# tmtlakmal/acme

Hardware: NVIDIA B200
Metric: learner_updates_per_sec_dqn_atari_b256 (higher is better)
Workload: dtype bf16 tensor-core operands (activations, weight shadows, back-propagated gradients), f32 accumulate, f32 master weights, weight gradients and optimizer

## Files before the change

acme_b200/_capi.py:

```python

from __future__ import annotations

import ctypes as C
import os

_LIB_PATH = os.path.join(os.path.dirname(os.path.abspath(__file__)), 'lib', 'libb200rl.so')

c_i32, c_i64, c_u64, c_f32, c_f64, c_vp, c_int = (C.c_int32, C.c_int64, C.c_uint64, C.c_float,
                                                  C.c_double, C.c_void_p, C.c_int)


class ReplayCfg(C.Structure):
  _fields_ = [('max_items', c_i64), ('slot_capacity', c_i64), ('obs_bytes', c_i32),
              ('act_bytes', c_i32), ('max_window', c_i32), ('shard_count', c_i32),
              ('shard_rank', c_i32), ('device', c_i32), ('stage_slots', c_i32),
              ('frame_stack', c_i32), ('gamma', c_f32), ('reserved_f', c_f32), ('alpha', c_f64)]


class DpCfg(C.Structure):
  _fields_ = [('world', c_i32), ('rank', c_i32), ('device', c_i32), ('reserved', c_i32), ('n_params', c_i64)]


class ConvGeom(C.Structure):
  _fields_ = [(n, c_i32) for n in ('B', 'H', 'W', 'C', 'kh', 'kw', 'stride', 'pad_top',
# ... 65 lines not shown
                                  c_int, c_vp, c_i64, c_vp]),
    'b200rl_linear_dgrad': (c_int, [c_i32, c_i32, c_i32, c_vp, c_i32, c_vp, c_vp, c_i32, c_vp, c_int,
                                    c_int, c_vp, c_i64, c_vp]),
    'b200rl_linear_wgrad': (c_int, [c_i32, c_i32, c_i32, c_vp, c_i32, c_vp, c_i32, c_vp, c_vp, c_int,
                                    c_vp, c_i64, c_vp]),
    'b200rl_act_bwd': (c_int, [c_i64, c_vp, c_vp, c_int, c_vp]),
    'b200rl_duelling_fwd': (c_int, [c_i32, c_i32, c_vp, c_vp, c_vp, c_vp]),
    'b200rl_duelling_bwd': (c_int, [c_i32, c_i32, c_vp, c_vp, c_vp, c_vp]),
    'b200rl_duelling_head_fwd': (c_int, [c_i32, c_i32, c_i32, c_vp, c_i32, c_vp, c_vp, c_vp, c_vp, c_vp, c_vp, c_vp, c_vp]),
    'b200rl_duelling_head_bwd': (c_int, [c_i32, c_i32, c_i32, c_vp, c_vp, c_i32, c_vp, c_vp, c_vp, c_vp, c_vp, c_i32, c_vp, c_vp,
                                          c_vp, c_vp, c_vp, c_i64, c_vp]),
    'b200rl_dqn_head_td': (c_int, [c_i32, c_i32, c_i32, c_vp, c_vp, c_vp, c_i32, c_vp, c_vp, c_vp, c_vp, c_vp, c_vp, c_vp, c_vp,
                                   c_vp, c_vp, c_vp, c_vp, c_f32, c_f32, c_f64, c_f32, c_vp, c_f32, c_i32, c_vp, c_vp, c_vp, c_vp,
                                   c_vp, c_vp, c_vp, c_vp, c_vp, c_vp, c_vp, c_i32, c_i32, c_vp]),
    'b200rl_mean': (c_int, [c_i32, c_vp, c_vp, c_vp]),
    'b200rl_duelling_head_wgrad': (c_int, [c_i32, c_i32, c_i32, c_vp, c_vp, c_vp, c_i32, c_vp, c_vp, c_vp, c_vp, c_vp, c_i64, c_vp]),
    'b200rl_bf16_from_f32': (c_int, [c_i64, c_vp, c_vp, c_vp]),
    'b200rl_conv2d_rows_bf16_bytes': (c_i64, [C.POINTER(ConvGeom)]),
    'b200rl_conv2d_rows_bf16_from_u8': (c_int, [c_vp, C.POINTER(ConvGeom), c_vp, c_i64, c_vp]),
    'b200rl_conv2d_fwd_bf16': (c_int, [c_vp, c_int, c_vp, c_vp, c_vp, c_int, C.POINTER(ConvGeom), c_int, c_vp, c_i64, c_vp]),
    'b200rl_conv2d_wgrad_bf16': (c_int, [c_vp, c_int, c_vp, c_vp, c_vp, C.POINTER(ConvGeom), c_vp, c_i64, c_vp]),
    'b200rl_conv2d_dgrad_bf16': (c_int, [c_vp, c_vp, c_vp, c_int, C.POINTER(ConvGeom), c_vp, c_int, c_int, c_vp]),
    'b200rl_linear_fwd_bf16': (c_int, [c_i32, c_i32, c_i32, c_vp, c_i32, c_vp, c_vp, c_vp, c_i32, c_int, c_int, c_vp, c_i64, c_vp]),
    'b200rl_linear_dgrad_bf16': (c_int, [c_i32, c_i32, c_i32, c_vp, c_i32, c_vp, c_vp, c_i32, c_int, c_vp, c_int, c_int, c_vp,
                                         c_i64, c_vp]),
    'b200rl_colsum_bf16': (c_int, [c_i32, c_i32, c_vp, c_i32, c_vp, c_vp, c_i64, c_vp]),
    'b200rl_linear_wgrad_bf16': (c_int, [c_i32, c_i32, c_i32, c_vp, c_i32, c_vp, c_i32, c_vp, c_vp, c_vp, c_i64, c_vp]),
    'b200rl_layernorm_tanh_fwd': (c_int, [c_i32, c_i32, c_vp, c_vp, c_vp, c_f32, c_vp, c_vp, c_vp, c_vp]),
    'b200rl_layernorm_tanh_bwd': (c_int, [c_i32, c_i32, c_vp, c_vp, c_vp, c_vp, c_vp, c_vp, c_vp, c_vp, c_vp]),
    'b200rl_tanh_to_spec_fwd': (c_int, [c_i32, c_i32, c_vp, c_vp, c_vp, c_vp, c_vp]),
    'b200rl_tanh_to_spec_bwd': (c_int, [c_i32, c_i32, c_vp, c_vp, c_vp, c_vp, c_vp]),
    'b200rl_concat2': (c_int, [c_i32, c_i32, c_i32, c_vp, c_vp, c_vp, c_vp]),
    'b200rl_split_second': (c_int, [c_i32, c_i32, c_i32, c_vp, c_vp, c_vp]),
    'b200rl_workspace_bytes': (c_i64, [c_i64]),
    'b200rl_conv2d_rows_bytes': (c_i64, [C.POINTER(ConvGeom)]),
    'b200rl_conv2d_rows_from_u8': (c_int, [c_vp, C.POINTER(ConvGeom), c_vp, c_i64, c_vp]),
    'b200rl_dp_create': (c_int, [C.POINTER(c_vp), C.POINTER(DpCfg)]),
    'b200rl_dp_destroy': (c_int, [c_vp]),
    'b200rl_dp_buffers': (c_int, [c_vp, C.POINTER(c_vp), C.POINTER(c_vp)]),
    'b200rl_dp_export': (c_int, [c_vp, c_vp]),
    'b200rl_dp_import': (c_int, [c_vp, c_i32, c_vp]),
    'b200rl_dp_max_f64': (c_int, [c_vp, c_vp, c_vp, c_vp]),
    'b200rl_dp_adam': (c_int, [c_vp, c_i64, c_i64, c_vp, c_vp, c_vp, C.c_float, C.c_double, C.c_double, C.c_float, c_int,
                               c_i32, c_i32, c_vp]),
    'b200rl_dp_reduce_adam_ce': (c_int, [c_vp, c_i64, c_i64, c_vp, c_vp, c_vp, C.c_float, C.c_double, C.c_double, C.c_float, c_int,
                                 c_i32, c_vp, c_i32, c_vp]),
    'b200rl_dp_region_bytes': (c_i64, [c_i64]),
    'b200rl_dp_create_external': (c_int, [C.POINTER(c_vp), C.POINTER(DpCfg), C.POINTER(c_vp), c_vp]),
# ... 71 lines not shown
```

acme_b200/csrc/gemm_bf16.cu:

```cuda
#include <algorithm>
#include <cstdlib>

#include <cuda.h>
#include <cuda_bf16.h>

#include "common.cuh"
#include "gemm_common.cuh"
#include "tc_common.cuh"
#include "tma_common.cuh"

namespace b200rl {

typedef __nv_bfloat16 bf16;
constexpr int HBM_ROWS = 128, H_THREADS = 192;

__device__ unsigned long long* g_h_timeline = nullptr;
__device__ __forceinline__ void h_mark(int slot, int cta) {
  if (g_h_timeline && (int)(blockIdx.x + blockIdx.y * gridDim.x) == cta && blockIdx.z == 0) {
    unsigned long long t;
    asm volatile("mov.u64 %0, %%globaltimer;" : "=l"(t));
    g_h_timeline[slot] = t;
  }
}

// ... 415 lines not shown
      rc = launch_h_pers<KE, BM, BN, true>(ma, mb, epi, M, N, K, kps, splits, res_b, stream, conv);
    else
      rc = launch_h_pers<KE, BM, BN, false>(ma, mb, epi, M, N, K, kps, splits, 0, stream, conv);
    if (rc) return rc;
    if (splits > 1) return launch_splitk_finish(epi, M, N, splits, stream);
    return B200RL_OK;
  }
  dim3 grid(ceil_div(N, BN), ceil_div(M, HBM_ROWS), splits);
  constexpr int smem = STAGES * STAGE + 1024;
  static bool attr = false;
  if (!attr) {
    B200RL_CUDA_OK(cudaFuncSetAttribute(hgemm_kernel<KE, AM, BM, BN, STAGES>, cudaFuncAttributeMaxDynamicSharedMemorySize, smem));
    attr = true;
  }
  epi.pdl_late = pdl_late_mode();
  B200RL_CUDA_OK(launch_pdl(hgemm_kernel<KE, AM, BM, BN, STAGES>, grid, dim3(H_THREADS), smem, stream, ma, mb, epi, M, N, K, kps, conv));
  B200RL_LAUNCH_OK();
  if (splits > 1) return launch_splitk_finish(epi, M, N, splits, stream);
  return B200RL_OK;
}
static const ConvA kNoConv{0, 0, 0, 0, 0, 0, 0, 0, 0, 0};
static int bn_for(int N) { return N <= 32 ? 32 : (N <= 64 ? 64 : 128); }

static Epilogue make_epi(void* out, int ldo, const float* bias, int act, const void* mask, int ldmask, int mask_act,
                         int transpose, int out_bf16, int mask_bf16, float scale) {
  Epilogue e{(float*)out, ldo, bias, act, (const float*)mask, ldmask, mask_act, nullptr, transpose, out_bf16, mask_bf16, scale};
  return e;
}

int h_linear_fwd(int M, int N, int K, const bf16* x, int ldx, const bf16* w, const float* bias, void* y, int ldy, int act,
                 int out_bf16, void* ws, int64_t wsb, cudaStream_t s) {
  if (!ok16(x, ldx) || !ok16(w, K) || K < 64) return 1;
  const int BN = bn_for(N);
  CUtensorMap ma, mb;
  if (!make_map_h(&ma, x, M, K, ldx, 64, HBM_ROWS) || !make_map_h(&mb, w, N, K, K, 64, BN)) return 1;
  Epilogue e = make_epi(y, ldy, bias, act, nullptr, 0, 0, 0, out_bf16, 0, 0.f);
  if (BN == 32) return launch_h<64, 0, 0, 32>(ma, mb, e, M, N, K, ws, wsb, s, kNoConv);
  if (BN == 64) return launch_h<64, 0, 0, 64>(ma, mb, e, M, N, K, ws, wsb, s, kNoConv);
  return launch_h<64, 0, 0, 128>(ma, mb, e, M, N, K, ws, wsb, s, kNoConv);
}
int h_linear_dgrad(int M, int N, int K, const bf16* dy, int lddy, const bf16* w, void* dx, int lddx, const void* mask,
                   int ldmask, int mask_act, int out_bf16, int mask_bf16, void* ws, int64_t wsb, cudaStream_t s) {
  if (!ok16(dy, lddy) || !ok16(w, K) || N < 64 || K % 64 != 0) return 1;
  int BN = K >= 128 ? 128 : 64;
  if (BN == 128 && ceil_div(M, HBM_ROWS) * ceil_div(K, 128) < kNumSMs) BN = 64;
  CUtensorMap ma, mb;
  if (!make_map_h(&ma, dy, M, N, lddy, 64, HBM_ROWS) || !make_map_h(&mb, w, N, K, K, 64, 64)) return 1;
  Epilogue e = make_epi(dx, lddx, nullptr, 0, mask, ldmask, mask_act, 0, out_bf16, mask_bf16, 0.f);
  return BN == 64 ? launch_h<64, 0, 1, 64>(ma, mb, e, M, K, N, ws, wsb, s, kNoConv, false)
                  : launch_h<64, 0, 1, 128>(ma, mb, e, M, K, N, ws, wsb, s, kNoConv, false);
}
int launch_colsum_bf16(int M, int N, const bf16* x, int ld, float* out, void* ws, int64_t ws_bytes, cudaStream_t stream);

int h_linear_wgrad(int M, int N, int K, const bf16* dy, int lddy, const bf16* x, int ldx, float* dw, float* db, void* ws,
                   int64_t wsb, cudaStream_t s) {
  if (!ok16(dy, lddy) || !ok16(x, ldx) || N % 64 != 0 || K % 64 != 0) return 1;
  const int BN = K >= 128 ? 128 : 64;
  CUtensorMap ma, mb;
  if (!make_map_h(&ma, dy, M, N, lddy, 64, 64) || !make_map_h(&mb, x, M, K, ldx, 64, 64)) return 1;
  Epilogue e = make_epi(dw, K, nullptr, 0, nullptr, 0, 0, 0, 0, 0, 0.f);
  int rc = BN == 64 ? launch_h<64, 1, 1, 64>(ma, mb, e, N, K, M, ws, wsb, s, kNoConv)
                    : launch_h<64, 1, 1, 128>(ma, mb, e, N, K, M, ws, wsb, s, kNoConv);
  if (rc) return rc;
  if (db) return launch_colsum_bf16(M, N, dy, lddy, db, ws, wsb, s);
  return B200RL_OK;
}

int h_conv_fwd(const bf16* x, const bf16* w, const float* bias, void* y, const b200rl_conv_geom& g, int act, int out_bf16,
               void* ws, int64_t wsb, cudaStream_t s) {
  const int M = g.B * g.OH * g.OW, K = g.kh * g.kw * g.C;
  if ((g.C != 32 && g.C % 64 != 0) || !ok16(x, g.C) || !ok16(w, K) || (g.Cout != 32 && g.Cout != 64 && g.Cout != 128)) return 1;
  const int KE = g.C == 32 ? 32 : 64;
  CUtensorMap ma, mb;
// ... 490 lines not shown
```

acme_b200/csrc/layers_api.cu:

```cuda
#include <cuda_bf16.h>

#include "common.cuh"

namespace b200rl {
int simt_linear_fwd(int M, int N, int K, const float* x, int ldx, const float* w, const float* bias, float* y,
                    int ldy, int act, void* ws, int64_t wsb, cudaStream_t s);
int simt_linear_dgrad(int M, int N, int K, const float* dy, int lddy, const float* w, float* dx, int lddx,
                      const float* mask, int ldmask, int mask_act, void* ws, int64_t wsb, cudaStream_t s);
int simt_linear_wgrad(int M, int N, int K, const float* dy, int lddy, const float* x, int ldx, float* dw, float* db,
                      void* ws, int64_t wsb, cudaStream_t s);
int simt_conv_fwd(const void* x, int x_u8, const float* w, const float* bias, float* y, const b200rl_conv_geom& g,
                  int act, void* ws, int64_t wsb, cudaStream_t s);
int simt_conv_wgrad(const void* x, int x_u8, const float* dy, float* dw, float* db, const b200rl_conv_geom& g,
                    void* ws, int64_t wsb, cudaStream_t s);
int simt_conv_dgrad(const float* dy, const float* w, float* dx, const b200rl_conv_geom& g, const float* mask,
                    int mask_act, void* ws, int64_t wsb, cudaStream_t s);
int tc_linear_fwd(int M, int N, int K, const float* x, int ldx, const float* w, const float* bias, float* y,
                  int ldy, int act, void* ws, int64_t wsb, cudaStream_t s);
int tc_linear_dgrad(int M, int N, int K, const float* dy, int lddy, const float* w, float* dx, int lddx,
                    const float* mask, int ldmask, int mask_act, void* ws, int64_t wsb, cudaStream_t s);
int tc_linear_wgrad(int M, int N, int K, const float* dy, int lddy, const float* x, int ldx, float* dw, float* db,
                    void* ws, int64_t wsb, cudaStream_t s);
int tc_conv_fwd(const void* x, int x_u8, const float* w, const float* bias, float* y, const b200rl_conv_geom& g,
                int act, void* ws, int64_t wsb, cudaStream_t s);
// ... 5 lines not shown
                   int ldy, int act, void* ws, int64_t wsb, cudaStream_t s);
int tma_linear_dgrad(int M, int N, int K, const float* dy, int lddy, const float* w, float* dx, int lddx,
                     const float* mask, int ldmask, int mask_act, void* ws, int64_t wsb, cudaStream_t s);
int tma_linear_wgrad(int M, int N, int K, const float* dy, int lddy, const float* x, int ldx, float* dw, float* db,
                     void* ws, int64_t wsb, cudaStream_t s);
int tma_conv_fwd(const float* x, const float* w, const float* bias, float* y, const b200rl_conv_geom& g, int act,
                 void* ws, int64_t wsb, cudaStream_t s);
int tma_conv_wgrad(const float* x, const float* dy, float* dw, float* db, const b200rl_conv_geom& g, void* ws, int64_t wsb,
                   cudaStream_t s);
int tma_conv_dgrad(const float* dy, const float* w, float* dx, const b200rl_conv_geom& g, const float* mask, int mask_act,
                   void* ws, int64_t wsb, cudaStream_t s);
int tma_conv_fwd_u8(const uint8_t* x, const float* w, const float* bias, float* y, const b200rl_conv_geom& g, int act,
                    void* ws, int64_t wsb, cudaStream_t s);
int tma_conv_wgrad_u8(const uint8_t* x, const float* dy, float* dw, float* db, const b200rl_conv_geom& g, void* ws, int64_t wsb,
                      cudaStream_t s);
int64_t tma_rows_bytes(const b200rl_conv_geom& g);
int tma_rows_from_u8(const uint8_t* x, const b200rl_conv_geom& g, float* rows, int64_t bytes, cudaStream_t s);
int tma_conv_fwd_rows(const float* rows, const float* w, const float* bias, float* y, const b200rl_conv_geom& g, int act,
                      void* ws, int64_t wsb, cudaStream_t s);
int tma_conv_wgrad_rows(const float* rows, const float* dy, float* dw, float* db, const b200rl_conv_geom& g, void* ws,
                        int64_t wsb, cudaStream_t s);
int h_linear_fwd(int M, int N, int K, const __nv_bfloat16* x, int ldx, const __nv_bfloat16* w, const float* bias, void* y, int ldy,
                 int act, int out_bf16, void* ws, int64_t wsb, cudaStream_t s);
int h_linear_dgrad(int M, int N, int K, const __nv_bfloat16* dy, int lddy, const __nv_bfloat16* w, void* dx, int lddx,
                   const void* mask, int ldmask, int mask_act, int out_bf16, int mask_bf16, void* ws, int64_t wsb, cudaStream_t s);
int h_linear_wgrad(int M, int N, int K, const __nv_bfloat16* dy, int lddy, const __nv_bfloat16* x, int ldx, float* dw, float* db,
                   void* ws, int64_t wsb, cudaStream_t s);
int h_conv_fwd(const __nv_bfloat16* x, const __nv_bfloat16* w, const float* bias, void* y, const b200rl_conv_geom& g, int act,
               int out_bf16, void* ws, int64_t wsb, cudaStream_t s);
int h_conv_wgrad(const __nv_bfloat16* x, const __nv_bfloat16* dy, float* dw, float* db, const b200rl_conv_geom& g, void* ws,
                 int64_t wsb, cudaStream_t s);
int h_conv_dgrad(const __nv_bfloat16* dy, const __nv_bfloat16* w, void* dx, const b200rl_conv_geom& g, const void* mask,
                 int mask_act, int out_bf16, int mask_bf16, cudaStream_t s);
int64_t h_rows_bytes(const b200rl_conv_geom& g);
int h_rows_from_u8(const uint8_t* x, const b200rl_conv_geom& g, __nv_bfloat16* rows, int64_t bytes, cudaStream_t s);
int h_conv_fwd_rows(const __nv_bfloat16* rows, const __nv_bfloat16* w, const float* bias, void* y, const b200rl_conv_geom& g,
                    int act, int out_bf16, void* ws, int64_t wsb, cudaStream_t s);
int h_conv_wgrad_rows(const __nv_bfloat16* rows, const __nv_bfloat16* dy, float* dw, float* db, const b200rl_conv_geom& g,
                      void* ws, int64_t wsb, cudaStream_t s);
int h_f32_to_bf16(int64_t n, const float* src, __nv_bfloat16* dst, cudaStream_t s);
int launch_colsum_bf16(int M, int N, const __nv_bfloat16* x, int ld, float* out, void* ws, int64_t ws_bytes, cudaStream_t stream);
}

using namespace b200rl;

static bool g_use_tma = true;
static inline int small_dense(int precision, int M, int N, int K) {
  return (precision == 1 && (long long)M * N * K < (1ll << 26)) ? 0 : precision;
// ... 149 lines not shown
  H_CALL(h_conv_fwd((const bf16_t*)x, (const bf16_t*)w, bias, y, *g, act, y_bf16, ws, wsb, as_stream(stream)), "conv2d_fwd_bf16");
}
extern "C" int b200rl_conv2d_wgrad_bf16(const void* x, int x_rows, const void* dy, float* dw, float* db, const b200rl_conv_geom* g,
                                        void* ws, int64_t wsb, void* stream) {
  B200RL_REQUIRE(x && dy && dw && ws, "null argument");
  if (int rc = check_geom(g)) return rc;
  if (x_rows)
    H_CALL(h_conv_wgrad_rows((const bf16_t*)x, (const bf16_t*)dy, dw, db, *g, ws, wsb, as_stream(stream)), "conv2d_wgrad_bf16(rows)");
  H_CALL(h_conv_wgrad((const bf16_t*)x, (const bf16_t*)dy, dw, db, *g, ws, wsb, as_stream(stream)), "conv2d_wgrad_bf16");
}
extern "C" int b200rl_conv2d_dgrad_bf16(const void* dy, const void* w, void* dx, int dx_bf16, const b200rl_conv_geom* g,
                                        const void* mask_y, int mask_bf16, int mask_act, void* stream) {
  B200RL_REQUIRE(dy && w && dx, "null argument");
  if (int rc = check_geom(g)) return rc;
  H_CALL(h_conv_dgrad((const bf16_t*)dy, (const bf16_t*)w, dx, *g, mask_y, mask_act, dx_bf16, mask_bf16, as_stream(stream)),
         "conv2d_dgrad_bf16");
}
extern "C" int b200rl_linear_fwd_bf16(int32_t M, int32_t N, int32_t K, const void* x, int32_t ldx, const void* w, const float* bias,
                                      void* y, int32_t ldy, int y_bf16, int act, void* ws, int64_t wsb, void* stream) {
  B200RL_REQUIRE(x && w && y && M >= 1 && N >= 1 && K >= 1 && ldx >= K && ldy >= N, "bad argument");
  H_CALL(h_linear_fwd(M, N, K, (const bf16_t*)x, ldx, (const bf16_t*)w, bias, y, ldy, act, y_bf16, ws, wsb, as_stream(stream)),
         "linear_fwd_bf16");
}
extern "C" int b200rl_linear_dgrad_bf16(int32_t M, int32_t N, int32_t K, const void* dy, int32_t lddy, const void* w, void* dx,
                                        int32_t lddx, int dx_bf16, const void* mask_y, int mask_bf16, int mask_act, void* ws,
                                        int64_t wsb, void* stream) {
  B200RL_REQUIRE(dy && w && dx && M >= 1 && N >= 1 && K >= 1 && lddy >= N && lddx >= K, "bad argument");
  H_CALL(h_linear_dgrad(M, N, K, (const bf16_t*)dy, lddy, (const bf16_t*)w, dx, lddx, mask_y, lddx, mask_act, dx_bf16, mask_bf16, ws,
                        wsb, as_stream(stream)),
         "linear_dgrad_bf16");
}
extern "C" int b200rl_linear_wgrad_bf16(int32_t M, int32_t N, int32_t K, const void* dy, int32_t lddy, const void* x, int32_t ldx,
                                        float* dw, float* db, void* ws, int64_t wsb, void* stream) {
  B200RL_REQUIRE(dy && x && dw && ws && M >= 1 && N >= 1 && K >= 1 && lddy >= N && ldx >= K, "bad argument");
  H_CALL(h_linear_wgrad(M, N, K, (const bf16_t*)dy, lddy, (const bf16_t*)x, ldx, dw, db, ws, wsb, as_stream(stream)),
         "linear_wgrad_bf16");
}

extern "C" int b200rl_colsum_bf16(int32_t M, int32_t N, const void* x_bf16, int32_t ld, float* out, void* ws, int64_t wsb,
                                  void* stream) {
  B200RL_REQUIRE(x_bf16 && out && ws && M >= 1 && N >= 1 && ld >= N, "bad argument");
  return launch_colsum_bf16(M, N, (const bf16_t*)x_bf16, ld, out, ws, wsb, as_stream(stream));
}
```

acme_b200/networks.py:

```python

from __future__ import annotations

import math
from typing import Dict, List, Optional, Tuple

import numpy as np

from acme_b200 import _capi
from acme_b200._capi import ACT_ELU, ACT_NONE, ACT_RELU, ACT_TANH, ConvGeom


def tf_same_pad(size: int, k: int, s: int) -> Tuple[int, int]:
  out = -(-size // s)
  total = max((out - 1) * s + k - size, 0)
  return out, total // 2


def _truncated_normal(rng, shape, std):
  x = rng.standard_normal(shape)
  bad = np.abs(x) > 2
  while bad.any():
    x[bad] = rng.standard_normal(int(bad.sum()))
    bad = np.abs(x) > 2
  return (x * std).astype(np.float32)
# ... 290 lines not shown
    _capi.call(name, obs.data_ptr(), self.geom(0, B), buf.data_ptr(), buf.numel(), _capi.current_stream())
    return buf

  def features(self, obs, bufs, before_fc1=None, rows=None):
    import torch
    B, P, st = bufs['B'], self.params, _capi.current_stream()
    ws, wsb = self.ws
    if self.flow:
      P.ensure_shadow()
      if rows is None:
        if obs.dtype != torch.uint8:
          raise ValueError('the bf16 dataflow reads uint8 frames')
        rows = self.prepare_frames(obs, 'fwd')
      x, x_rows = rows.data_ptr(), 1
      self._mark(f'fwd{B}.start')
      for i in range(3):
        y = bufs[f'y{i + 1}']
        _capi.call('b200rl_conv2d_fwd_bf16', x, x_rows, P.sp(f'conv{i + 1}.w'), P.p(f'conv{i + 1}.b'), y.data_ptr(), 1,
                   self.geom(i, B), ACT_RELU, ws, wsb, st)
        self._mark(f'fwd{B}.conv{i + 1}')
        x, x_rows = y.data_ptr(), 0
      if before_fc1 is not None:
        before_fc1()
      _capi.call('b200rl_linear_fwd_bf16', B, 1024, self.flat_dim, x, self.flat_dim, P.sp('fc1.w'), P.p('fc1.b'),
                 bufs['h'].data_ptr(), 1024, 0, ACT_RELU, ws, wsb, st)
      self._mark(f'fwd{B}.fc1')
      return bufs['h']
    x, x_u8 = obs.data_ptr(), int(obs.dtype == torch.uint8)
    if rows is not None:
      x, x_u8 = rows.data_ptr(), 2
    for i in range(3):
      y = bufs[f'y{i + 1}']
      g = self.geom(i, B)
      _capi.call('b200rl_conv2d_fwd', x, x_u8, P.p(f'conv{i + 1}.w'), P.p(f'conv{i + 1}.b'), y.data_ptr(),
                 g, ACT_RELU, self.precision, ws, wsb, st)
      x, x_u8 = y.data_ptr(), 0
    if before_fc1 is not None:
      before_fc1()
    h = bufs['h']
    _linear(B, 1024, self.flat_dim, x, self.flat_dim, P.p('fc1.w'), P.p('fc1.b'), h.data_ptr(), 1024, ACT_RELU, self)
    return h

  def head_params(self):
    P = self.params
    return P.p('v2.w'), P.p('v2.b'), P.p('a2.w'), P.p('a2.b')

  def forward(self, obs, bufs, before_fc1=None, rows=None) -> 'torch.Tensor':
    P, B = self.params, bufs['B']
# ... 17 lines not shown
    ws, wsb = self.ws
    _capi.call('b200rl_duelling_head_wgrad', B, self.A, 512, gbufs['dval'].data_ptr(), gbufs['dadv'].data_ptr(),
               bufs['h'].data_ptr(), 1024, P.g('v2.w'), P.g('v2.b'), P.g('a2.w'), P.g('a2.b'), ws, wsb, _capi.current_stream())

  def _fc1_bias_grad(self, bufs, gbufs):
    B, P = bufs['B'], self.params
    ws, wsb = self.ws
    _capi.call('b200rl_colsum_bf16', B, 1024, gbufs['dh'].data_ptr(), 1024, P.g('fc1.b'), ws, wsb, _capi.current_stream())

  def _fc1_wgrad(self, bufs, gbufs, bias: bool = True):
    B, P = bufs['B'], self.params
    ws, wsb = self.ws
    if self.flow:
      _capi.call('b200rl_linear_wgrad_bf16', B, 1024, self.flat_dim, gbufs['dh'].data_ptr(), 1024, bufs['y3'].data_ptr(),
                 self.flat_dim, P.g('fc1.w'), P.g('fc1.b') if bias else None, ws, wsb, _capi.current_stream())
    else:
      _linear_wgrad(B, 1024, self.flat_dim, gbufs['dh'].data_ptr(), 1024, bufs['y3'].data_ptr(), self.flat_dim, P.g('fc1.w'),
                    P.g('fc1.b'), self)

  def _fc1_dgrad(self, bufs, gbufs):
    B, P = bufs['B'], self.params
    ws, wsb = self.ws
    if self.flow:
      _capi.call('b200rl_linear_dgrad_bf16', B, 1024, self.flat_dim, gbufs['dh'].data_ptr(), 1024, P.sp('fc1.w'),
                 gbufs['dy3'].data_ptr(), self.flat_dim, 1, bufs['y3'].data_ptr(), 1, ACT_RELU, ws, wsb, _capi.current_stream())
    else:
      _linear_dgrad(B, 1024, self.flat_dim, gbufs['dh'].data_ptr(), 1024, P.p('fc1.w'), gbufs['dy3'].data_ptr(), self.flat_dim,
                    bufs['y3'].data_ptr(), ACT_RELU, self)

  def _conv_bias_grad(self, i, bufs, gbufs):
    B, P = bufs['B'], self.params
    ws, wsb = self.ws
    _, _, _, co, _, oh, _ = self.convs[i]
    _capi.call('b200rl_colsum_bf16', B * oh * oh, co, gbufs[f'dy{i + 1}'].data_ptr(), co, P.g(f'conv{i + 1}.b'), ws, wsb,
               _capi.current_stream())

  def _conv_wgrad(self, i, obs, bufs, gbufs, rows, bias: bool = True):
    import torch
    B, P = bufs['B'], self.params
    ws, wsb = self.ws
    g = self.geom(i, B)
    dy = gbufs[f'dy{i + 1}'].data_ptr()
    if self.flow:
      if i > 0:
        x, x_rows = bufs[f'y{i}'].data_ptr(), 0
      else:
        if rows is None:
          rows = self.prepare_frames(obs, 'bwd')
# ... 379 lines not shown
```

include/b200rl.h:

```cpp
#ifndef B200RL_H_
#define B200RL_H_

#include <stdint.h>

#ifdef __cplusplus
extern "C" {
#endif

#define B200RL_VERSION 100

#define B200RL_OK 0
#define B200RL_EINVAL (-1)
#define B200RL_ECUDA (-2)
#define B200RL_EAGAIN (-3)
#define B200RL_EARCH (-4)

int b200rl_version(void);
uint64_t b200rl_launch_count(void);
const char* b200rl_last_error(void);
int b200rl_device_check(int device);

typedef struct b200rl_replay b200rl_replay;

typedef struct b200rl_replay_cfg {
// ... 169 lines not shown
                       const int32_t* a_tm1, const float* R, const float* D, const float* prob, float gamma,
                       float huber_delta, double is_exponent, float max_abs_reward, const double* wmax_dev,
                       float grad_scale, int32_t flags, float* q_tm1, float* q_t_value, float* q_t_selector, float* td,
                       float* loss_per_sample, float* weight, float* priority, float* dq_tm1, float* dvalue, float* dadv,
                       void* dh, int32_t lddh, int32_t dh_bf16, void* stream);
int b200rl_mean(int32_t n, const float* x, float* out, void* stream);
int b200rl_duelling_head_wgrad(int32_t B, int32_t A, int32_t H, const float* dvalue, const float* dadv, const float* h,
                               int32_t ldh, float* dwv, float* dbv, float* dwa, float* dba, void* ws, int64_t ws_bytes,
                               void* stream);

int b200rl_bf16_from_f32(int64_t n, const float* src, void* dst_bf16, void* stream);
int64_t b200rl_conv2d_rows_bf16_bytes(const b200rl_conv_geom* g);
int b200rl_conv2d_rows_bf16_from_u8(const void* x_u8, const b200rl_conv_geom* g, void* rows_bf16, int64_t rows_bytes,
                                    void* stream);
int b200rl_conv2d_fwd_bf16(const void* x, int x_rows, const void* w_bf16, const float* bias, void* y, int y_bf16,
                           const b200rl_conv_geom* g, int act, void* ws, int64_t ws_bytes, void* stream);
int b200rl_conv2d_wgrad_bf16(const void* x, int x_rows, const void* dy_bf16, float* dw, float* db,
                             const b200rl_conv_geom* g, void* ws, int64_t ws_bytes, void* stream);
int b200rl_conv2d_dgrad_bf16(const void* dy_bf16, const void* w_bf16, void* dx, int dx_bf16, const b200rl_conv_geom* g,
                             const void* mask_y, int mask_bf16, int mask_act, void* stream);
int b200rl_linear_fwd_bf16(int32_t M, int32_t N, int32_t K, const void* x_bf16, int32_t ldx, const void* w_bf16,
                           const float* bias, void* y, int32_t ldy, int y_bf16, int act, void* ws, int64_t ws_bytes,
                           void* stream);
int b200rl_linear_dgrad_bf16(int32_t M, int32_t N, int32_t K, const void* dy_bf16, int32_t lddy, const void* w_bf16,
                             void* dx, int32_t lddx, int dx_bf16, const void* mask_y, int mask_bf16, int mask_act,
                             void* ws, int64_t ws_bytes, void* stream);
int b200rl_colsum_bf16(int32_t M, int32_t N, const void* x_bf16, int32_t ld, float* out, void* ws, int64_t ws_bytes,
                       void* stream);
int b200rl_linear_wgrad_bf16(int32_t M, int32_t N, int32_t K, const void* dy_bf16, int32_t lddy, const void* x_bf16,
                             int32_t ldx, float* dw, float* db, void* ws, int64_t ws_bytes, void* stream);

typedef struct b200rl_dp* b200rl_dp_t;
typedef struct b200rl_dp_cfg {
  int32_t world, rank, device, reserved;
  int64_t n_params;
} b200rl_dp_cfg;
int b200rl_dp_create(b200rl_dp_t* out, const b200rl_dp_cfg* cfg);
int b200rl_dp_destroy(b200rl_dp_t h);
int b200rl_dp_buffers(b200rl_dp_t h, float** params, float** grads);
int b200rl_dp_export(b200rl_dp_t h, void* handle64);
int b200rl_dp_import(b200rl_dp_t h, int32_t peer_rank, const void* handle64);
int b200rl_dp_max_f64(b200rl_dp_t h, double* value_dev, const int64_t* step_dev, void* stream);
int b200rl_dp_adam(b200rl_dp_t h, int64_t off, int64_t n, float* m, float* v, const int64_t* step_dev, float lr,
                   double b1, double b2, float eps, int eps_mode, int32_t bucket, int32_t final_barrier, void* stream);
int b200rl_dp_status(b200rl_dp_t h);
int64_t b200rl_dp_region_bytes(int64_t n_params);
int b200rl_dp_create_external(b200rl_dp_t* out, const b200rl_dp_cfg* cfg, void* const* bases, void* multicast_base);
int b200rl_dp_has_multicast(b200rl_dp_t h);
int b200rl_dp_adam_mc(b200rl_dp_t h, int64_t off, int64_t n, float* m, float* v, const int64_t* step_dev, float lr,
// ... 20 lines not shown
```

Baseline: 3661.

## Add cluster-based split-K fc1 forward and multicast dgrad kernels

Adds a split-K forward GEMM for fc1 whose K-splits form one thread-block cluster. Partial accumulators are reduced through distributed shared memory instead of a global workspace plus a separate finish kernel. Adds a dgrad kernel that multicasts the shared dy tile across a 4-CTA cluster via TMA, cutting redundant global loads. Both are wired into the DQN torso's fc1 forward and backward, at the cost of cluster scheduling constraints and a smaller per-CTA N tile in dgrad.

```diff
diff --git a/acme_b200/_capi.py b/acme_b200/_capi.py
--- a/acme_b200/_capi.py
+++ b/acme_b200/_capi.py
@@ -111,8 +111,11 @@
     'b200rl_conv2d_wgrad_bf16': (c_int, [c_vp, c_int, c_vp, c_vp, c_vp, C.POINTER(ConvGeom), c_vp, c_i64, c_vp]),
     'b200rl_conv2d_dgrad_bf16': (c_int, [c_vp, c_vp, c_vp, c_int, C.POINTER(ConvGeom), c_vp, c_int, c_int, c_vp]),
     'b200rl_linear_fwd_bf16': (c_int, [c_i32, c_i32, c_i32, c_vp, c_i32, c_vp, c_vp, c_vp, c_i32, c_int, c_int, c_vp, c_i64, c_vp]),
+    'b200rl_linear_fwd_bf16_cluster': (c_int, [c_i32, c_i32, c_i32, c_vp, c_i32, c_vp, c_vp, c_vp, c_i32, c_int, c_int, c_vp]),
     'b200rl_linear_dgrad_bf16': (c_int, [c_i32, c_i32, c_i32, c_vp, c_i32, c_vp, c_vp, c_i32, c_int, c_vp, c_int, c_int, c_vp,
                                          c_i64, c_vp]),
+    'b200rl_linear_dgrad_bf16_cluster': (c_int, [c_i32, c_i32, c_i32, c_vp, c_i32, c_vp, c_vp, c_i32, c_int, c_vp, c_int, c_int,
+                                                 c_vp]),
     'b200rl_colsum_bf16': (c_int, [c_i32, c_i32, c_vp, c_i32, c_vp, c_vp, c_i64, c_vp]),
     'b200rl_linear_wgrad_bf16': (c_int, [c_i32, c_i32, c_i32, c_vp, c_i32, c_vp, c_i32, c_vp, c_vp, c_vp, c_i64, c_vp]),
     'b200rl_layernorm_tanh_fwd': (c_int, [c_i32, c_i32, c_vp, c_vp, c_vp, c_f32, c_vp, c_vp, c_vp, c_vp]),
diff --git a/acme_b200/csrc/gemm_bf16.cu b/acme_b200/csrc/gemm_bf16.cu
--- a/acme_b200/csrc/gemm_bf16.cu
+++ b/acme_b200/csrc/gemm_bf16.cu
@@ -461,6 +461,151 @@
 static const ConvA kNoConv{0, 0, 0, 0, 0, 0, 0, 0, 0, 0};
 static int bn_for(int N) { return N <= 32 ? 32 : (N <= 64 ? 64 : 128); }
 
+constexpr int HC_CHUNKS = 32, HC_MAX_SPLITS = 16;
+__device__ __forceinline__ uint32_t cluster_addr(uint32_t saddr, uint32_t rank) {
+  uint32_t r;
+  asm volatile("mapa.shared::cluster.u32 %0, %1, %2;" : "=r"(r) : "r"(saddr), "r"(rank));
+  return r;
+}
+__device__ __forceinline__ void st_cluster_f4(uint32_t addr, float a, float b, float c, float d) {
+  asm volatile("st.shared::cluster.v4.f32 [%0], {%1, %2, %3, %4};" ::"r"(addr), "f"(a), "f"(b), "f"(c), "f"(d) : "memory");
+}
+__device__ __forceinline__ void cluster_sync() {
+  asm volatile("barrier.cluster.arrive.release;\n\tbarrier.cluster.wait.acquire;" ::: "memory");
+}
+
+template <int STAGES>
+__global__ void __launch_bounds__(H_THREADS)
+hgemm_cluster_kernel(const __grid_constant__ CUtensorMap map_a, const __grid_constant__ CUtensorMap map_b, Epilogue epi, int M,
+                     int N, int K, int kblocks_per_split) {
+  constexpr int KE = 64, BN = 128, A_BYTES = HBM_ROWS * KE * 2, STAGE = A_BYTES + BN * KE * 2;
+  constexpr int SLOT = HBM_ROWS * 16;
+  static_assert(STAGES * STAGE >= (HC_CHUNKS + HC_MAX_SPLITS - 1) * SLOT, "the receive slots reuse the drained pipeline stages");
+  extern __shared__ uint8_t smem_raw[];
+  const uint32_t base = (smem_u32(smem_raw) + 1023u) & ~1023u;
+  __shared__ __align__(8) uint64_t bar_full[STAGES], bar_empty[STAGES], bar_done;
+  __shared__ uint32_t tmem_base_smem;
+
+  const int tid = threadIdx.x, warp = tid >> 5, lane = tid & 31;
+  if (!epi.pdl_late) pdl_launch_dependents();
+  const int row0 = blockIdx.y * HBM_ROWS, col0 = blockIdx.x * BN;
+  const int S = gridDim.z, split = blockIdx.z;
+  const int ncl = (HC_CHUNKS + S - 1) / S;
+  const int total_kblocks = (K + KE - 1) / KE;
+  const int kb_begin = split * kblocks_per_split;
+  const int nkb = min(total_kblocks, kb_begin + kblocks_per_split) - kb_begin;
+
+  if (tid == 0) {
+    prefetch_tensormap(&map_a);
+    prefetch_tensormap(&map_b);
+#pragma unroll
+    for (int s = 0; s < STAGES; ++s) { mbar_init(&bar_full[s], 1); mbar_init(&bar_empty[s], 1); }
+    mbar_init(&bar_done, 1);
+    asm volatile("fence.mbarrier_init.release.cluster;" ::: "memory");
+  }
+  if (warp == 1) tmem_alloc(&tmem_base_smem, BN);
+  tc_fence_before();
+  __syncthreads();
+  tc_fence_after();
+  pdl_wait();
+  const uint32_t tmem_d = tmem_base_smem;
+
+  if (warp == 0 && lane == 0) {
+    for (int i = 0; i < nkb; ++i) {
+      const int s = i % STAGES;
+      if (i >= STAGES) mbar_wait(&bar_empty[s], ((i / STAGES) - 1) & 1);
+      const uint32_t sa = base + s * STAGE, sb = sa + A_BYTES;
+      const int k0 = (kb_begin + i) * KE;
+      mbar_expect_tx(&bar_full[s], STAGE);
+      tma_load_2d(sa, &map_a, k0, row0, &bar_full[s]);
+      tma_load_2d(sb, &map_b, k0, col0, &bar_full[s]);
+    }
+  } else if (warp == 1 && lane == 0) {
+    constexpr uint32_t idesc = idesc_bf16(HBM_ROWS, BN, false, false);
+    for (int i = 0; i < nkb; ++i) {
+      const int s = i % STAGES;
+      mbar_wait(&bar_full[s], (i / STAGES) & 1);
+      tc_fence_after();
+      const uint32_t sa = base + s * STAGE, sb = sa + A_BYTES;
+#pragma unroll
+      for (int kk = 0; kk < KE / 16; ++kk)
+        umma_bf16(tmem_d, operand_desc<0, KE>(sa, kk), operand_desc<0, KE>(sb, kk), idesc, (i > 0 || kk > 0) ? 1u : 0u);
+      umma_commit(&bar_empty[s]);
+      if (i == nkb - 1) umma_commit(&bar_done);
+    }
+  } else if (warp >= 2) {
+    if (nkb > 0) {
+      mbar_wait(&bar_done, 0);
+      tc_fence_after();
+    }
+    if (epi.pdl_late) pdl_launch_dependents();
+  }
+  cluster_sync();
+
+  const int r = (warp & 3) * 32 + lane;
+  const int row = row0 + r;
+  if (warp >= 2) {
+#pragma unroll
+    for (int cc = 0; cc < BN; cc += 32) {
+      float v[32];
+      if (nkb > 0) tmem_ld32(tmem_d + ((uint32_t)((warp & 3) * 32) << 16) + (uint32_t)cc, v);
+      else {
+#pragma unroll
+        for (int j = 0; j < 32; ++j) v[j] = 0.f;
+      }
+      if (row < M) {
+#pragma unroll
+        for (int q = 0; q < 8; ++q) {
+          const int c = cc / 4 + q;
+          const int o = (S * (c + 1) - 1) / HC_CHUNKS, j = c - (HC_CHUNKS * o) / S;
+          const uint32_t dst = cluster_addr(base + (uint32_t)(((split * ncl + j) * HBM_ROWS + r) * 16), (uint32_t)o);
+          st_cluster_f4(dst, v[4 * q], v[4 * q + 1], v[4 * q + 2], v[4 * q + 3]);
+        }
+      }
+    }
+  }
+  cluster_sync();
+
+  if (warp >= 2 && row < M) {
+    const float4* recv = reinterpret_cast<const float4*>(smem_raw + (base - smem_u32(smem_raw)));
+    const int first = (HC_CHUNKS * split) / S, cnt = (HC_CHUNKS * (split + 1)) / S - first;
+    const bool vec = !epi.out_bf16 && (epi.ldo & 3) == 0 && ((uintptr_t)epi.out & 15) == 0;
+    for (int j = 0; j < cnt; ++j) {
+      const int col = col0 + 4 * (first + j);
+      if (col >= N) break;
+      float4 a[4];
+#pragma unroll
+      for (int t = 0; t < 4; ++t) a[t] = make_float4(0.f, 0.f, 0.f, 0.f);
+      auto add = [&](float4& d, int s) {
+        const float4 p = recv[(s * ncl + j) * HBM_ROWS + r];
+        d.x += p.x; d.y += p.y; d.z += p.z; d.w += p.w;
+      };
+      int s = 0;
+      for (; s + 4 <= S; s += 4) { add(a[0], s); add(a[1], s + 1); add(a[2], s + 2); add(a[3], s + 3); }
+      if (s < S) add(a[0], s);
+      if (s + 1 < S) add(a[1], s + 1);
+      if (s + 2 < S) add(a[2], s + 2);
+      float v[4] = {(a[0].x + a[1].x) + (a[2].x + a[3].x), (a[0].y + a[1].y) + (a[2].y + a[3].y),
+                    (a[0].z + a[1].z) + (a[2].z + a[3].z), (a[0].w + a[1].w) + (a[2].w + a[3].w)};
+      if (vec && col + 3 < N) {
+#pragma unroll
+        for (int e = 0; e < 4; ++e) {
+          v[e] *= epi_scale(epi);
+          if (epi.bias) v[e] += epi.bias[col + e];
+          v[e] = apply_act(v[e], epi.act);
+        }
+        *reinterpret_cast<float4*>(epi.out + (size_t)row * epi.ldo + col) = make_float4(v[0], v[1], v[2], v[3]);
+      } else {
+#pragma unroll
+        for (int e = 0; e < 4; ++e) if (col + e < N) finish(epi, row, col + e, v[e]);
+      }
+    }
+  }
+  tc_fence_before();
+  __syncthreads();
+  if (warp == 1) tmem_dealloc(tmem_d, BN);
+}
+
 static Epilogue make_epi(void* out, int ldo, const float* bias, int act, const void* mask, int ldmask, int mask_act,
                          int transpose, int out_bf16, int mask_bf16, float scale) {
   Epilogue e{(float*)out, ldo, bias, act, (const float*)mask, ldmask, mask_act, nullptr, transpose, out_bf16, mask_bf16, scale};
@@ -478,6 +623,61 @@
   if (BN == 64) return launch_h<64, 0, 0, 64>(ma, mb, e, M, N, K, ws, wsb, s, kNoConv);
   return launch_h<64, 0, 0, 128>(ma, mb, e, M, N, K, ws, wsb, s, kNoConv);
 }
+int h_linear_fwd_cluster(int M, int N, int K, const bf16* x, int ldx, const bf16* w, const float* bias, void* y, int ldy, int act,
+                         int out_bf16, cudaStream_t s) {
+  if (!ok16(x, ldx) || !ok16(w, K) || K < 64) return 1;
+  constexpr int BN = 128, STAGES = 3, smem = STAGES * (HBM_ROWS + BN) * 64 * 2 + 1024;
+  const int tiles = ceil_div(M, HBM_ROWS) * ceil_div(N, BN), kblocks = ceil_div(K, 64);
+  static const int sk_occ = getenv("B200RL_SPLITK_OCC") ? atoi(getenv("B200RL_SPLITK_OCC")) : SPLITK_OCC_DEFAULT;
+  static const int sk_min = getenv("B200RL_SPLITK_MIN_KB") ? atoi(getenv("B200RL_SPLITK_MIN_KB")) : SPLITK_MIN_KB_DEFAULT;
+  static const int sk_max = getenv("B200RL_SPLITK_MAX") ? atoi(getenv("B200RL_SPLITK_MAX")) : SPLITK_MAX_DEFAULT;
+  int splits = 1;
+  if (2 * tiles <= kNumSMs && kblocks >= 16) {
+    splits = std::min(ceil_div(sk_occ * kNumSMs, tiles), kblocks / sk_min);
+    splits = std::max(1, std::min(splits, sk_max));
+  }
+  const int kps = ceil_div(kblocks, splits);
+  splits = ceil_div(kblocks, kps);
+  if (splits > HC_MAX_SPLITS) return 1;
+  CUtensorMap ma, mb;
+  if (!make_map_h(&ma, x, M, K, ldx, 64, HBM_ROWS) || !make_map_h(&mb, w, N, K, K, 64, BN)) return 1;
+  Epilogue e = make_epi(y, ldy, bias, act, nullptr, 0, 0, 0, out_bf16, 0, 0.f);
+  e.pdl_late = pdl_late_mode();
+
+  auto kernel = hgemm_cluster_kernel<STAGES>;
+  static bool attr = false;
+  if (!attr) {
+    B200RL_CUDA_OK(cudaFuncSetAttribute(kernel, cudaFuncAttributeMaxDynamicSharedMemorySize, smem));
+    B200RL_CUDA_OK(cudaFuncSetAttribute(kernel, cudaFuncAttributeNonPortableClusterSizeAllowed, 1));
+    attr = true;
+  }
+  cudaLaunchConfig_t cfg = {};
+  cfg.gridDim = dim3(ceil_div(N, BN), ceil_div(M, HBM_ROWS), splits);
+  cfg.blockDim = dim3(H_THREADS);
+  cfg.dynamicSmemBytes = smem;
+  cfg.stream = s;
+  cudaLaunchAttribute la[2];
+  la[0].id = cudaLaunchAttributeClusterDimension;
+  la[0].val.clusterDim.x = 1;
+  la[0].val.clusterDim.y = 1;
+  la[0].val.clusterDim.z = splits;
+  la[1].id = cudaLaunchAttributeProgrammaticStreamSerialization;
+  la[1].val.programmaticStreamSerializationAllowed = 1;
+  cfg.attrs = la;
+  cfg.numAttrs = 1;
+  static int schedulable[HC_MAX_SPLITS + 1] = {};
+  if (!schedulable[splits]) {
+    int n = 0;
+    B200RL_CUDA_OK(cudaOccupancyMaxActiveClusters(&n, kernel, &cfg));
+    schedulable[splits] = n > 0 ? 1 : -1;
+  }
+  B200RL_REQUIRE(schedulable[splits] > 0, "linear_fwd_bf16_cluster: a cluster of %d CTAs (%d B of shared memory each) cannot be scheduled",
+                 splits, smem);
+  cfg.numAttrs = pdl_enabled() ? 2 : 1;
+  B200RL_CUDA_OK(cudaLaunchKernelEx(&cfg, kernel, ma, mb, e, M, N, K, kps));
+  B200RL_LAUNCH_OK();
+  return B200RL_OK;
+}
 int h_linear_dgrad(int M, int N, int K, const bf16* dy, int lddy, const bf16* w, void* dx, int lddx, const void* mask,
                    int ldmask, int mask_act, int out_bf16, int mask_bf16, void* ws, int64_t wsb, cudaStream_t s) {
   if (!ok16(dy, lddy) || !ok16(w, K) || N < 64 || K % 64 != 0) return 1;
@@ -488,6 +688,141 @@
   Epilogue e = make_epi(dx, lddx, nullptr, 0, mask, ldmask, mask_act, 0, out_bf16, mask_bf16, 0.f);
   return BN == 64 ? launch_h<64, 0, 1, 64>(ma, mb, e, M, K, N, ws, wsb, s, kNoConv, false)
                   : launch_h<64, 0, 1, 128>(ma, mb, e, M, K, N, ws, wsb, s, kNoConv, false);
+}
+
+__device__ __forceinline__ void tma_load_2d_mc(uint32_t smem_dst, const CUtensorMap* map, int c0, int c1, uint64_t* bar, uint16_t mask) {
+  asm volatile(
+      "cp.async.bulk.tensor.2d.shared::cluster.global.mbarrier::complete_tx::bytes.multicast::cluster [%0], [%1, {%2, %3}], [%4], %5;"
+      ::"r"(smem_dst), "l"(reinterpret_cast<uint64_t>(map)), "r"(c0), "r"(c1), "r"(smem_u32(bar)), "h"(mask)
+      : "memory");
+}
+__device__ __forceinline__ void umma_commit_mc(uint64_t* bar, uint16_t mask) {
+  asm volatile("tcgen05.commit.cta_group::1.mbarrier::arrive::one.shared::cluster.multicast::cluster.b64 [%0], %1;"
+               ::"r"(smem_u32(bar)), "h"(mask) : "memory");
+}
+
+template <int CN>
+__global__ void __launch_bounds__(H_THREADS)
+hgemm_mc_kernel(const __grid_constant__ CUtensorMap map_a, const __grid_constant__ CUtensorMap map_b, Epilogue epi, int M, int N,
+                int K) {
+  constexpr int KE = 64, BN = 64, STAGES = 3, A_BYTES = HBM_ROWS * KE * 2, B_BYTES = BN * KE * 2, STAGE = A_BYTES + B_BYTES;
+  constexpr int SLICE_ROWS = 16, NSLICE = HBM_ROWS / SLICE_ROWS, SLICE_BYTES = SLICE_ROWS * KE * 2;
+  static_assert(NSLICE % CN == 0, "whole dy slices per CTA");
+  static_assert(STAGES * STAGE >= HBM_ROWS * BN * 4, "the epilogue slab reuses the drained pipeline stages");
+  extern __shared__ uint8_t smem_raw[];
+  const uint32_t base = (smem_u32(smem_raw) + 1023u) & ~1023u;
+  __shared__ __align__(8) uint64_t bar_full[STAGES], bar_empty[STAGES], bar_done;
+  __shared__ uint32_t tmem_base_smem;
+
+  const int tid = threadIdx.x, warp = tid >> 5, lane = tid & 31;
+  if (!epi.pdl_late) pdl_launch_dependents();
+  const int row0 = blockIdx.y * HBM_ROWS, col0 = blockIdx.x * BN;
+  const int rank = blockIdx.x % CN;
+  constexpr uint16_t peers = (uint16_t)((1u << CN) - 1);
+  const int nkb = (K + KE - 1) / KE;
+
+  if (tid == 0) {
+    prefetch_tensormap(&map_a);
+    prefetch_tensormap(&map_b);
+#pragma unroll
+    for (int s = 0; s < STAGES; ++s) { mbar_init(&bar_full[s], 1); mbar_init(&bar_empty[s], CN); }
+    mbar_init(&bar_done, 1);
+    asm volatile("fence.mbarrier_init.release.cluster;" ::: "memory");
+  }
+  if (warp == 1) tmem_alloc(&tmem_base_smem, BN);
+  tc_fence_before();
+  __syncthreads();
+  tc_fence_after();
+  cluster_sync();
+  pdl_wait();
+  const uint32_t tmem_d = tmem_base_smem;
+
+  if (warp == 0 && lane == 0) {
+    for (int i = 0; i < nkb; ++i) {
+      const int s = i % STAGES;
+      if (i >= STAGES) mbar_wait(&bar_empty[s], ((i / STAGES) - 1) & 1);
+      const uint32_t sa = base + s * STAGE, sb = sa + A_BYTES;
+      const int k0 = i * KE;
+      mbar_expect_tx(&bar_full[s], STAGE);
+#pragma unroll
+      for (int q = 0; q < NSLICE / CN; ++q) {
+        const int j = rank + q * CN;
+        tma_load_2d_mc(sa + j * SLICE_BYTES, &map_a, k0, row0 + j * SLICE_ROWS, &bar_full[s], peers);
+      }
+      tma_load_2d(sb, &map_b, col0, k0, &bar_full[s]);
+    }
+    for (int i = max(0, nkb - STAGES); i < nkb; ++i) mbar_wait(&bar_empty[i % STAGES], (i / STAGES) & 1);
+  } else if (warp == 1 && lane == 0) {
+    constexpr uint32_t idesc = idesc_bf16(HBM_ROWS, BN, false, true);
+    for (int i = 0; i < nkb; ++i) {
+      const int s = i % STAGES;
+      mbar_wait(&bar_full[s], (i / STAGES) & 1);
+      tc_fence_after();
+      const uint32_t sa = base + s * STAGE, sb = sa + A_BYTES;
+#pragma unroll
+      for (int kk = 0; kk < KE / 16; ++kk)
+        umma_bf16(tmem_d, operand_desc<0, KE>(sa, kk), operand_desc<1, KE>(sb, kk), idesc, (i > 0 || kk > 0) ? 1u : 0u);
+      umma_commit_mc(&bar_empty[s], peers);
+      if (i == nkb - 1) umma_commit(&bar_done);
+    }
+  } else if (warp >= 2) {
+    const int lane_base = (warp & 3) * 32;
+    const int first = row0 + lane_base;
+    auto row_of = [&](int r) -> long long { return first + r < M ? first + r : -1; };
+    uint2 pm[32 / (32 / (BN / 4))];
+    const bool have_pm = prefetch_relu_mask<BN>(epi, lane, col0, N, row_of, pm);
+    mbar_wait(&bar_done, 0);
+    tc_fence_after();
+    if (epi.pdl_late) pdl_launch_dependents();
+    float* slab = reinterpret_cast<float*>(smem_raw + (base - smem_u32(smem_raw))) + (warp & 3) * 32 * BN;
+    stage_accumulator<BN>(tmem_d + ((uint32_t)lane_base << 16), slab, lane, true);
+    store_staged_rows<BN>(epi, slab, lane, col0, N, M, row_of, have_pm ? pm : nullptr);
+  }
+  tc_fence_before();
+  __syncthreads();
+  cluster_sync();
+  if (warp == 1) tmem_dealloc(tmem_d, BN);
+}
+
+int h_linear_dgrad_cluster(int M, int N, int K, const bf16* dy, int lddy, const bf16* w, void* dx, int lddx, const void* mask,
+                           int ldmask, int mask_act, int out_bf16, int mask_bf16, cudaStream_t s) {
+  if (!ok16(dy, lddy) || !ok16(w, K) || N < 64 || K % 64 != 0) return 1;
+  constexpr int CN = 4, BN = 64, smem = 3 * (HBM_ROWS + BN) * 64 * 2 + 1024;
+  CUtensorMap ma, mb;
+  if (!make_map_h(&ma, dy, M, N, lddy, 64, 16) || !make_map_h(&mb, w, N, K, K, 64, 64)) return 1;
+  Epilogue e = make_epi(dx, lddx, nullptr, 0, mask, ldmask, mask_act, 0, out_bf16, mask_bf16, 0.f);
+  e.pdl_late = pdl_late_mode();
+  auto kernel = hgemm_mc_kernel<CN>;
+  static bool attr = false;
+  if (!attr) {
+    B200RL_CUDA_OK(cudaFuncSetAttribute(kernel, cudaFuncAttributeMaxDynamicSharedMemorySize, smem));
+    attr = true;
+  }
+  cudaLaunchConfig_t cfg = {};
+  cfg.gridDim = dim3(ceil_div(ceil_div(K, BN), CN) * CN, ceil_div(M, HBM_ROWS), 1);
+  cfg.blockDim = dim3(H_THREADS);
+  cfg.dynamicSmemBytes = smem;
+  cfg.stream = s;
+  cudaLaunchAttribute la[2];
+  la[0].id = cudaLaunchAttributeClusterDimension;
+  la[0].val.clusterDim.x = CN;
+  la[0].val.clusterDim.y = 1;
+  la[0].val.clusterDim.z = 1;
+  la[1].id = cudaLaunchAttributeProgrammaticStreamSerialization;
+  la[1].val.programmaticStreamSerializationAllowed = 1;
+  cfg.attrs = la;
+  cfg.numAttrs = 1;
+  static int schedulable = 0;
+  if (!schedulable) {
+    int n = 0;
+    B200RL_CUDA_OK(cudaOccupancyMaxActiveClusters(&n, kernel, &cfg));
+    schedulable = n > 0 ? 1 : -1;
+  }
+  B200RL_REQUIRE(schedulable > 0, "linear_dgrad_bf16_cluster: a cluster of %d CTAs cannot be scheduled", CN);
+  cfg.numAttrs = pdl_enabled() ? 2 : 1;
+  B200RL_CUDA_OK(cudaLaunchKernelEx(&cfg, kernel, ma, mb, e, M, K, N));
+  B200RL_LAUNCH_OK();
+  return B200RL_OK;
 }
 int launch_colsum_bf16(int M, int N, const bf16* x, int ld, float* out, void* ws, int64_t ws_bytes, cudaStream_t stream);
 
diff --git a/acme_b200/csrc/layers_api.cu b/acme_b200/csrc/layers_api.cu
--- a/acme_b200/csrc/layers_api.cu
+++ b/acme_b200/csrc/layers_api.cu
@@ -51,8 +51,12 @@
                         int64_t wsb, cudaStream_t s);
 int h_linear_fwd(int M, int N, int K, const __nv_bfloat16* x, int ldx, const __nv_bfloat16* w, const float* bias, void* y, int ldy,
                  int act, int out_bf16, void* ws, int64_t wsb, cudaStream_t s);
+int h_linear_fwd_cluster(int M, int N, int K, const __nv_bfloat16* x, int ldx, const __nv_bfloat16* w, const float* bias, void* y,
+                         int ldy, int act, int out_bf16, cudaStream_t s);
 int h_linear_dgrad(int M, int N, int K, const __nv_bfloat16* dy, int lddy, const __nv_bfloat16* w, void* dx, int lddx,
                    const void* mask, int ldmask, int mask_act, int out_bf16, int mask_bf16, void* ws, int64_t wsb, cudaStream_t s);
+int h_linear_dgrad_cluster(int M, int N, int K, const __nv_bfloat16* dy, int lddy, const __nv_bfloat16* w, void* dx, int lddx,
+                           const void* mask, int ldmask, int mask_act, int out_bf16, int mask_bf16, cudaStream_t s);
 int h_linear_wgrad(int M, int N, int K, const __nv_bfloat16* dy, int lddy, const __nv_bfloat16* x, int ldx, float* dw, float* db,
                    void* ws, int64_t wsb, cudaStream_t s);
 int h_conv_fwd(const __nv_bfloat16* x, const __nv_bfloat16* w, const float* bias, void* y, const b200rl_conv_geom& g, int act,
@@ -248,6 +252,12 @@
   H_CALL(h_linear_fwd(M, N, K, (const bf16_t*)x, ldx, (const bf16_t*)w, bias, y, ldy, act, y_bf16, ws, wsb, as_stream(stream)),
          "linear_fwd_bf16");
 }
+extern "C" int b200rl_linear_fwd_bf16_cluster(int32_t M, int32_t N, int32_t K, const void* x, int32_t ldx, const void* w,
+                                              const float* bias, void* y, int32_t ldy, int y_bf16, int act, void* stream) {
+  B200RL_REQUIRE(x && w && y && M >= 1 && N >= 1 && K >= 1 && ldx >= K && ldy >= N, "bad argument");
+  H_CALL(h_linear_fwd_cluster(M, N, K, (const bf16_t*)x, ldx, (const bf16_t*)w, bias, y, ldy, act, y_bf16, as_stream(stream)),
+         "linear_fwd_bf16_cluster (at most 16 splits)");
+}
 extern "C" int b200rl_linear_dgrad_bf16(int32_t M, int32_t N, int32_t K, const void* dy, int32_t lddy, const void* w, void* dx,
                                         int32_t lddx, int dx_bf16, const void* mask_y, int mask_bf16, int mask_act, void* ws,
                                         int64_t wsb, void* stream) {
@@ -256,6 +266,14 @@
                         wsb, as_stream(stream)),
          "linear_dgrad_bf16");
 }
+extern "C" int b200rl_linear_dgrad_bf16_cluster(int32_t M, int32_t N, int32_t K, const void* dy, int32_t lddy, const void* w,
+                                                void* dx, int32_t lddx, int dx_bf16, const void* mask_y, int mask_bf16, int mask_act,
+                                                void* stream) {
+  B200RL_REQUIRE(dy && w && dx && M >= 1 && N >= 1 && K >= 1 && lddy >= N && lddx >= K, "bad argument");
+  H_CALL(h_linear_dgrad_cluster(M, N, K, (const bf16_t*)dy, lddy, (const bf16_t*)w, dx, lddx, mask_y, lddx, mask_act, dx_bf16,
+                                mask_bf16, as_stream(stream)),
+         "linear_dgrad_bf16_cluster");
+}
 extern "C" int b200rl_linear_wgrad_bf16(int32_t M, int32_t N, int32_t K, const void* dy, int32_t lddy, const void* x, int32_t ldx,
                                         float* dw, float* db, void* ws, int64_t wsb, void* stream) {
   B200RL_REQUIRE(dy && x && dw && ws && M >= 1 && N >= 1 && K >= 1 && lddy >= N && ldx >= K, "bad argument");
diff --git a/acme_b200/networks.py b/acme_b200/networks.py
--- a/acme_b200/networks.py
+++ b/acme_b200/networks.py
@@ -336,8 +336,8 @@
         x, x_rows = y.data_ptr(), 0
       if before_fc1 is not None:
         before_fc1()
-      _capi.call('b200rl_linear_fwd_bf16', B, 1024, self.flat_dim, x, self.flat_dim, P.sp('fc1.w'), P.p('fc1.b'),
-                 bufs['h'].data_ptr(), 1024, 0, ACT_RELU, ws, wsb, st)
+      _capi.call('b200rl_linear_fwd_bf16_cluster', B, 1024, self.flat_dim, x, self.flat_dim, P.sp('fc1.w'), P.p('fc1.b'),
+                 bufs['h'].data_ptr(), 1024, 0, ACT_RELU, st)
       self._mark(f'fwd{B}.fc1')
       return bufs['h']
     x, x_u8 = obs.data_ptr(), int(obs.dtype == torch.uint8)
@@ -401,8 +401,8 @@
     B, P = bufs['B'], self.params
     ws, wsb = self.ws
     if self.flow:
-      _capi.call('b200rl_linear_dgrad_bf16', B, 1024, self.flat_dim, gbufs['dh'].data_ptr(), 1024, P.sp('fc1.w'),
-                 gbufs['dy3'].data_ptr(), self.flat_dim, 1, bufs['y3'].data_ptr(), 1, ACT_RELU, ws, wsb, _capi.current_stream())
+      _capi.call('b200rl_linear_dgrad_bf16_cluster', B, 1024, self.flat_dim, gbufs['dh'].data_ptr(), 1024, P.sp('fc1.w'),
+                 gbufs['dy3'].data_ptr(), self.flat_dim, 1, bufs['y3'].data_ptr(), 1, ACT_RELU, _capi.current_stream())
     else:
       _linear_dgrad(B, 1024, self.flat_dim, gbufs['dh'].data_ptr(), 1024, P.p('fc1.w'), gbufs['dy3'].data_ptr(), self.flat_dim,
                     bufs['y3'].data_ptr(), ACT_RELU, self)
diff --git a/include/b200rl.h b/include/b200rl.h
--- a/include/b200rl.h
+++ b/include/b200rl.h
@@ -215,9 +215,14 @@
 int b200rl_linear_fwd_bf16(int32_t M, int32_t N, int32_t K, const void* x_bf16, int32_t ldx, const void* w_bf16,
                            const float* bias, void* y, int32_t ldy, int y_bf16, int act, void* ws, int64_t ws_bytes,
                            void* stream);
+int b200rl_linear_fwd_bf16_cluster(int32_t M, int32_t N, int32_t K, const void* x_bf16, int32_t ldx, const void* w_bf16,
+                                   const float* bias, void* y, int32_t ldy, int y_bf16, int act, void* stream);
 int b200rl_linear_dgrad_bf16(int32_t M, int32_t N, int32_t K, const void* dy_bf16, int32_t lddy, const void* w_bf16,
                              void* dx, int32_t lddx, int dx_bf16, const void* mask_y, int mask_bf16, int mask_act,
                              void* ws, int64_t ws_bytes, void* stream);
+int b200rl_linear_dgrad_bf16_cluster(int32_t M, int32_t N, int32_t K, const void* dy_bf16, int32_t lddy, const void* w_bf16,
+                                     void* dx, int32_t lddx, int dx_bf16, const void* mask_y, int mask_bf16, int mask_act,
+                                     void* stream);
 int b200rl_colsum_bf16(int32_t M, int32_t N, const void* x_bf16, int32_t ld, float* out, void* ws, int64_t ws_bytes,
                        void* stream);
 int b200rl_linear_wgrad_bf16(int32_t M, int32_t N, int32_t K, const void* dy_bf16, int32_t lddy, const void* x_bf16,
```

Measured after the change: 3726 (median of 6 runs). +1.8%, better.
